# fritzsedlazeck/Sniffles

Measured on AMD Instinct MI355X. Metric: SV-signatures clustered/sec (clustering + calling + QC + genotype + INS consensus), higher is better.
Workload: dtype int32/f64

## Files before the change

sniffles_amd/csrc/snf_fused.h:

```cpp
#pragma once
#include "snf_stage_final.h"
#include "snf_stage_cluster.h"
#include "snf_stage_call.h"

namespace snf {

template <int K>
SNF_D void block_exscan256(const unsigned long long (&val)[K], unsigned long long (&excl)[K], unsigned long long (&tot)[K],
                           unsigned long long* lds) {
  const int tid = threadIdx.x, lane = tid & 63, wid = tid >> 6;
  unsigned long long incl[K];
#pragma unroll
  for (int k = 0; k < K; k++) {
    unsigned long long x = val[k];
#pragma unroll
    for (int d = 1; d < 64; d <<= 1) { const unsigned long long y = __shfl_up(x, d, 64); if (lane >= d) x += y; }
    incl[k] = x;
    if (lane == 63) lds[wid * K + k] = x;
  }
  __syncthreads();
#pragma unroll
  for (int k = 0; k < K; k++) {
    unsigned long long base = 0, all = 0;
#pragma unroll
// ... 165 lines not shown
  if (p < n) {
    v.headscan[p] = (uint32_t)off[0];
    if (p == n - 1) { const int64_t nb = (int64_t)(off[0] + val[0]); v.headscan[n] = (uint32_t)nb; v.cnt->n_bins = nb; v.bin_lo[nb] = (int32_t)v.cnt->n_valid; }
    a3_emit(p, v);
  }
}
SNF_FUSED_HEAD(a4k_binstats)
  if (p < n) a4_binstats_body(p, v);
  unsigned long long val[1] = {p < n ? (unsigned long long)v.eligflag[p] : 0ull};
  tile_publish<1>(v, TS_SEEDS, val, lds);
}
SNF_FUSED_HEAD(a7k_seeds)
  unsigned long long val[1] = {p < n ? (unsigned long long)v.eligflag[p] : 0ull}, off[1];
  tile_scan<1>(v, TS_SEEDS, val, off, lds);
  if (p < n) {
    v.eligscan[p] = (uint32_t)off[0];
    if (p == n - 1) { v.eligscan[n] = (uint32_t)(off[0] + val[0]); v.cnt->n_seeds = (int64_t)(off[0] + val[0]); }
    a7_seeds_body(p, v);
  }
}
SNF_FUSED_HEAD(a5k_leadflags)
  if (p < n) a5_leadflags_body(p, v);
  unsigned long long val[2] = {p < n ? (unsigned long long)v.fN[p] : 0ull, p < n ? (unsigned long long)v.fL[p] : 0ull};
  tile_publish<2>(v, TS_LEADS, val, lds);
}
SNF_FUSED_HEAD(a6k_scatter)
  unsigned long long val[2] = {p < n ? (unsigned long long)v.fN[p] : 0ull, p < n ? (unsigned long long)v.fL[p] : 0ull}, off[2];
  tile_scan<2>(v, TS_LEADS, val, off, lds);
  if (p < n) {
    v.pN[p] = (uint32_t)off[0]; v.pL[p] = (uint32_t)off[1];
    if (p == n - 1) {
      v.pN[n] = (uint32_t)(off[0] + val[0]); v.pL[n] = (uint32_t)(off[1] + val[1]);
      v.cnt->NF = (int64_t)(off[0] + val[0]); v.cnt->NLL = (int64_t)(off[1] + val[1]);
    }
    a6_emit(p, v);
  }
}
SNF_FUSED_HEAD(b1k_seedmetrics)
  if (p < n) b1_seedmetrics_body(p, v);
  unsigned long long val[1] = {p < n ? (unsigned long long)v.runflag[p] : 0ull};
  tile_publish<1>(v, TS_RUNS, val, lds);
}
SNF_FUSED_HEAD(b2k_runs)
  unsigned long long val[1] = {p < n ? (unsigned long long)v.runflag[p] : 0ull}, off[1];
  tile_scan<1>(v, TS_RUNS, val, off, lds);
  if (p < n) {
    v.runscan[p] = (uint32_t)off[0];
    if (p == n - 1) { const int64_t nr = (int64_t)(off[0] + val[0]); v.runscan[n] = (uint32_t)nr; v.cnt->n_runs = nr; v.run_first[nr] = (int32_t)v.cnt->n_seeds; }
    b2_emit(p, v);
  }
}
SNF_FUSED_HEAD(c4a_count)
  unsigned long long val[1] = {p < n ? (unsigned long long)v.clflag[p] : 0ull};
  tile_publish<1>(v, TS_CLUSTERS, val, lds);
}
SNF_FUSED_HEAD(c4k_clusters)
  unsigned long long val[1] = {p < n ? (unsigned long long)v.clflag[p] : 0ull}, off[1];
  tile_scan<1>(v, TS_CLUSTERS, val, off, lds);
  if (p < n) {
    v.clscan[p] = (uint32_t)off[0];
    if (p == n - 1) { v.clscan[n] = (uint32_t)(off[0] + val[0]); v.cnt->n_clusters = (int64_t)(off[0] + val[0]); }
    c4_emit(p, v);
  }
}
SNF_FUSED_HEAD(d1bk_rctable)
  unsigned long long val[1] = {p < n ? (unsigned long long)v.rcflag[p] : 0ull}, off[1];
  tile_scan_direct<1>(v, TS_REFINED, val, off, lds);
  if (p < n) {
    v.rcscan[p] = (uint32_t)off[0];
    if (p == n - 1) { v.rcscan[n] = (uint32_t)(off[0] + val[0]); v.cnt->n_rc = (int64_t)(off[0] + val[0]); }
    d1b_emit(p, v);
  }
}
SNF_FUSED_HEAD(d3ck_compact)
  unsigned long long val[1] = {(p < n && p < v.cnt->n_rc) ? (unsigned long long)v.cdflag[p] : 0ull}, off[1];
  tile_scan_direct<1>(v, TS_CALLS, val, off, lds);
  if (p < n) {
    v.cdscan[p] = (uint32_t)off[0];
    if (p == n - 1) { v.cdscan[n] = (uint32_t)(off[0] + val[0]); v.cnt->n_calls = (int64_t)(off[0] + val[0]); }
    d3_compact_emit(p, v);
  }
}

SNF_FUSED_HEAD(d3sk_svid)
  if (p < n) d3_svid_body(p, v);
  unsigned long long val[1] = {p < n ? (unsigned long long)v.rnf[p] : 0ull};
  tile_publish<1>(v, TS_RNAMES, val, lds);
}
SNF_FUSED_HEAD(d3rk_rnames)
  unsigned long long val[1] = {p < n ? (unsigned long long)v.rnf[p] : 0ull}, off[1];
  tile_scan<1>(v, TS_RNAMES, val, off, lds);
  if (p < n) {
    v.rnp[p] = (uint32_t)off[0];
    if (p == n - 1) { const int64_t tot = (int64_t)(off[0] + val[0]); v.rnp[n] = (uint32_t)tot; v.cnt->rn_total = tot; *v.res_rn_total = tot; }
    if (!v.rn_defer) d3_rnames_emit(p, v);
  }
}

SNF_CHAIN_HEAD(b12c_seedruns, TS_RUNS)
  if (p < n) b1_seedmetrics_body(p, v);
  unsigned long long val[1] = {p < n ? (unsigned long long)v.runflag[p] : 0ull}, off[1], tot[1];
  chain_scan<1>(v, TS_RUNS, tile, val, off, tot, lds);
  if (p < n) {
    v.runscan[p] = (uint32_t)off[0];
    if (p == n - 1) { const int64_t nr = (int64_t)tot[0]; v.runscan[n] = (uint32_t)nr; v.cnt->n_runs = nr; v.run_first[nr] = (int32_t)v.cnt->n_seeds; }
    b2_emit(p, v);
  }
}
SNF_CHAIN_HEAD(c4c_clusters, TS_CLUSTERS)
  unsigned long long val[1] = {p < n ? (unsigned long long)v.clflag[p] : 0ull}, off[1], tot[1];
  chain_scan<1>(v, TS_CLUSTERS, tile, val, off, tot, lds);
  if (p < n) {
    v.clscan[p] = (uint32_t)off[0];
    if (p == n - 1) { v.clscan[n] = (uint32_t)tot[0]; v.cnt->n_clusters = (int64_t)tot[0]; }
    c4_emit(p, v);
  }
}
SNF_CHAIN_HEAD(d1bc_rctable, TS_REFINED)
  unsigned long long val[1] = {p < n ? (unsigned long long)v.rcflag[p] : 0ull}, off[1], tot[1];
  chain_scan<1>(v, TS_REFINED, tile, val, off, tot, lds);
  if (p < n) {
    v.rcscan[p] = (uint32_t)off[0];
    if (p == n - 1) { v.rcscan[n] = (uint32_t)tot[0]; v.cnt->n_rc = (int64_t)tot[0]; }
    d1b_emit(p, v);
  }
}
SNF_CHAIN_HEAD(d3cc_compact, TS_CALLS)
  unsigned long long val[1] = {(p < n && p < v.cnt->n_rc) ? (unsigned long long)v.cdflag[p] : 0ull}, off[1], tot[1];
  chain_scan<1>(v, TS_CALLS, tile, val, off, tot, lds);
  if (p < n) {
    v.cdscan[p] = (uint32_t)off[0];
    if (p == n - 1) { v.cdscan[n] = (uint32_t)tot[0]; v.cnt->n_calls = (int64_t)tot[0]; }
    d3_compact_emit(p, v);
  }
}
SNF_CHAIN_HEAD(d3src_svid_rnames, TS_RNAMES)
  if (p < n) d3_svid_body(p, v);
  unsigned long long val[1] = {p < n ? (unsigned long long)v.rnf[p] : 0ull}, off[1], tot[1];
  chain_scan<1>(v, TS_RNAMES, tile, val, off, tot, lds);
  if (p < n) {
    v.rnp[p] = (uint32_t)off[0];
    if (p == n - 1) { v.rnp[n] = (uint32_t)tot[0]; v.cnt->rn_total = (int64_t)tot[0]; *v.res_rn_total = (int64_t)tot[0]; }
    if (!v.rn_defer) d3_rnames_emit(p, v);
  }
}

#define SNF_ALT_K 5
SNF_D void alt_values(const View& v, int64_t i, int64_t nc, unsigned long long (&val)[SNF_ALT_K]) {
  if (i < nc) { val[0] = v.fN[i]; val[1] = v.fL[i]; val[2] = (unsigned long long)v.sz_tab[i]; val[3] = (unsigned long long)v.sz_aln[i]; val[4] = (unsigned long long)v.sz_rd[i]; }
  else { for (int k = 0; k < SNF_ALT_K; k++) val[k] = 0; }
}
__global__ void __launch_bounds__(256) e2a_sizes(const View v, int64_t n_unused) {
  __shared__ unsigned long long lds[4 * SNF_ALT_K];
  const int64_t nc = v.cnt->n_calls;
  const int64_t i = (int64_t)blockIdx.x * 256 + threadIdx.x;
  for (int64_t k = i; k < 4 * 64 * 16; k += (int64_t)gridDim.x * 256) v.stripes[k] = 0;
  e2_best_body(i, v);
  unsigned long long val[SNF_ALT_K], excl[SNF_ALT_K], tot[SNF_ALT_K];
  alt_values(v, i, nc, val);
  block_exscan256<SNF_ALT_K>(val, excl, tot, lds);
  if (threadIdx.x == 0) for (int k = 0; k < SNF_ALT_K; k++) v.tile_sums[(int64_t)k * v.tile_stride + blockIdx.x] = tot[k];
}
__global__ void __launch_bounds__(256) e3b_offsets(const View v, int64_t n_unused) {
  IT_SCOPE(8)
  __shared__ unsigned long long lds[4 * SNF_ALT_K];
  const int64_t nc = v.cnt->n_calls;
  const int64_t i = (int64_t)blockIdx.x * 256 + threadIdx.x;
  if ((int64_t)blockIdx.x * 256 >= nc) return;
  unsigned long long part[SNF_ALT_K], dummy[SNF_ALT_K], prefix[SNF_ALT_K];
#pragma unroll
  for (int k = 0; k < SNF_ALT_K; k++) {
    unsigned long long a = 0;
    for (int64_t j = threadIdx.x; j < (int64_t)blockIdx.x; j += 256) a += v.tile_sums[(int64_t)k * v.tile_stride + j];
    part[k] = a;
  }
  block_exscan256<SNF_ALT_K>(part, dummy, prefix, lds);
  unsigned long long val[SNF_ALT_K], excl[SNF_ALT_K], tot[SNF_ALT_K];
  alt_values(v, i, nc, val);
  block_exscan256<SNF_ALT_K>(val, excl, tot, lds);
  if (i < nc) {
    const unsigned long long o0 = prefix[0] + excl[0], o1 = prefix[1] + excl[1], o2 = prefix[2] + excl[2], o3 = prefix[3] + excl[3],
                             o4 = prefix[4] + excl[4];
    v.pN[i] = (uint32_t)o0; v.pL[i] = (uint32_t)o1; v.sc_tab[i] = (int64_t)o2; v.sc_aln[i] = (int64_t)o3; v.sc_rd[i] = (int64_t)o4;
    if (i == nc - 1) {
      v.pN[nc] = (uint32_t)(o0 + val[0]); v.pL[nc] = (uint32_t)(o1 + val[1]);
      v.sc_tab[nc] = (int64_t)(o2 + val[2]); v.sc_aln[nc] = (int64_t)(o3 + val[3]); v.sc_rd[nc] = (int64_t)(o4 + val[4]);
      v.cnt->alt_total = (int64_t)(o0 + val[0]); v.cnt->n_cons = (int64_t)(o1 + val[1]);
      v.cnt->tab_total = (int64_t)(o2 + val[2]); v.cnt->aln_total = (int64_t)(o3 + val[3]); v.cnt->n_cons_reads = (int64_t)(o4 + val[4]);
      alt_decide(v, (int64_t)(o0 + val[0]));
    }
    e3_emit(i, v);
  }
}

}
```

sniffles_amd/csrc/snf_knobs.h:

```cpp
#pragma once
#include <climits>
#include <cstdlib>
#include <cstring>
#include <string>

namespace snf {

constexpr int KNOB_UNSET = INT_MIN;
inline bool env_set(const char* name) { return getenv(name) != nullptr; }
inline int env_int(const char* name, int unset) { const char* e = getenv(name); return e ? atoi(e) : unset; }
inline int env_pos(const char* name, int other) { const int v = env_int(name, 0); return v > 0 ? v : other; }
inline bool env_on(const char* name) { return env_int(name, 0) != 0; }
inline bool env_is(const char* name, const char* value) { const char* e = getenv(name); return e && strcmp(e, value) == 0; }
inline std::string env_str(const char* name) { const char* e = getenv(name); return e ? e : ""; }

struct BatchKnobs {
  bool wave_path = !env_set("SNF_NO_WAVE");
  bool fuse = !env_set("SNF_NO_FUSE");
  bool sort64 = env_set("SNF_SORT64");
  bool prefilter = !env_set("SNF_NO_PREFILTER");
  bool pf_spread = env_int("SNF_PF_SPREAD", 0) == 1;
  bool winfront = !env_set("SNF_NO_WINFRONT");
  int win_bits = env_int("SNF_WIN_BITS", 0);
  int win_bits_max = [] { const int v = env_int("SNF_WIN_BITS_MAX", 10); return v >= 6 && v <= 12 ? v : 10; }();
  bool w4_split = env_on("SNF_W4_SPLIT");
  bool pool_slices = !env_set("SNF_NO_POOL_SLICES");
  int fuse_copy = env_set("SNF_FUSE_COPY") ? env_on("SNF_FUSE_COPY") : -1;
  bool merge_reread = env_on("SNF_MERGE_REREAD");
  int run_gap = env_int("SNF_RUN_GAP", KNOB_UNSET);
  int chain = env_set("SNF_CHAIN") ? env_on("SNF_CHAIN") : env_set("SNF_NO_CHAIN") ? 0 : -1;
  int graph = env_set("SNF_GRAPH") ? env_on("SNF_GRAPH") : env_set("SNF_NO_GRAPH") ? 0 : -1;
  int heavy_n = env_int("SNF_HEAVY_N", 24);
  int e1_batch = env_int("SNF_E1_BATCH", 64);
  bool big_stage = !env_set("SNF_NO_BIG_STAGE");
  bool cov_exact = env_set("SNF_COV_EXACT");
  bool d4_thread = env_is("SNF_D4", "thread");
  bool d1_groups = !env_set("SNF_NO_D1_GROUPS");
  bool d2_groups = !env_set("SNF_NO_D2_GROUPS");
  bool d2_mid = env_set("SNF_D2_MID");
  bool rn_defer = !env_set("SNF_NO_RN_DEFER");
  bool rn_fuse = !env_set("SNF_NO_RN_FUSE");
  int grid_mult = env_int("SNF_GRID_MULT", 2);
  int grid_div = env_pos("SNF_GRID_DIV", 1);
  int occ_d2 = env_int("SNF_OCC_D2", 5);
  int occ_e1 = env_int("SNF_OCC_E1", 5);
  int occ_s = env_int("SNF_OCC_S", 5);
  int cons_nw = env_int("SNF_CONS_NW", 1);
  int cons_large_nw = env_int("SNF_CONS_LARGE_NW", 4);
  int cons_grid_mult = env_int("SNF_CONS_GRID_MULT", KNOB_UNSET);
  int cons_small_grid = env_pos("SNF_CONS_SMALL_GRID", 65536);
  int cons_order = env_int("SNF_CONS_ORDER", -1);
  bool serial = env_set("SNF_SERIAL");
  int f4_grid = env_pos("SNF_F4_GRID", 2048);
  bool large_prio = env_on("SNF_LARGE_PRIO");
  int readprep = env_int("SNF_READPREP", 1);
  bool readprep_each_pass = env_set("SNF_READPREP_EACH_PASS");
  int stage_out = env_int("SNF_STAGE_OUT", -1);
  bool stage_copy_kernel = env_is("SNF_STAGE_COPY", "kernel");
  bool alt_hbm = env_set("SNF_ALT_HBM");
  bool prof = env_set("SNF_PROF");
  bool timing = !env_set("SNF_NO_TIMING");
  bool timeline = env_set("SNF_TIMELINE");
  bool time_all = env_set("SNF_TIME_ALL");
  int time_every = env_int("SNF_TIME_EVERY", 8);
  std::string wg_trace_file = env_str("SNF_WG_TRACE_FILE");
};

struct ProcessKnobs {
  int pace = env_int("SNF_PACE", 1);
  double pace_frac = getenv("SNF_PACE_FRAC") ? atof(getenv("SNF_PACE_FRAC")) : 0.25;
  bool chain_gate = env_on("SNF_CHAIN_GATE");
  int gpu_slots = env_int("SNF_GPU_SLOTS", 0);
  size_t stage_arena_floor = getenv("SNF_STAGE_ARENA_MB") ? (size_t)atoll(getenv("SNF_STAGE_ARENA_MB")) << 20 : 0;
  bool slab_cache = !env_set("SNF_NO_SLAB_CACHE");
  bool stream_pool = !env_set("SNF_NO_STREAM_POOL");
  bool roctx = env_on("SNF_ROCTX");
  int upload_threads = env_set("SNF_UPLOAD_THREADS") ? env_pos("SNF_UPLOAD_THREADS", 1) : 0;
};
inline const ProcessKnobs& process_knobs() { static const ProcessKnobs k; return k; }

struct ExtractKnobs {
  bool thread_form = env_set("SNF_EXTRACT_THREAD");
  int waves = env_int("SNF_EXTRACT_WAVES", 4);
  int grid_cap = env_set("SNF_EXTRACT_GRID") ? env_pos("SNF_EXTRACT_GRID", 1) : (1 << 22);
  bool xtrace_emit = env_is("SNF_XTRACE_PASS", "emit");
  std::string xtrace_out = env_str("SNF_XTRACE_OUT");
};

struct BgzfKnobs {
  bool thread_form = env_set("SNF_BGZF_THREAD");
  int grid_cap = env_set("SNF_BGZF_GRID") ? env_pos("SNF_BGZF_GRID", 1) : (1 << 20);
};

struct BaiKnobs {
  bool thread_form = env_set("SNF_BAI_THREAD");
  int grid_cap = env_set("SNF_BAI_GRID") ? env_pos("SNF_BAI_GRID", 1) : (1 << 20);
};

struct DeflateKnobs {
  int grid_cap = env_set("SNF_DEFLATE_GRID") ? env_pos("SNF_DEFLATE_GRID", 1) : (1 << 20);
  int max_bits = [] { const int v = env_int("SNF_DEFLATE_MAXBITS", 15); return v >= 9 && v <= 15 ? v : 15; }();
};

struct FastaKnobs {
  int grid_cap = env_set("SNF_FASTA_GRID") ? env_pos("SNF_FASTA_GRID", 1) : (1 << 20);
};

struct CombineKnobs {
  bool thread_form = env_set("SNF_COMBINE_THREAD");
};

}
```

sniffles_amd/csrc/snf_lib.hip:

```cpp
#include "snf_stage_final.h"
#include "snf_wave_refine.h"
#include "snf_wave_cons.h"
#include "snf_fused.h"
#include "snf_stage_window.h"
#include "snf_stage_out.h"
#include "snf_wave_call.h"
#include "snf_wave_call_g.h"
#include "snf_wave_refine_g.h"
#include "snf_ctx.h"

#include <rocprim/device/device_radix_sort.hpp>
#include <rocprim/device/device_scan.hpp>

#include <fcntl.h>
#include <sys/file.h>
#include <unistd.h>

#include <atomic>
#include <map>
#include <tuple>
#include <cmath>
#include <ctime>
#include <memory>
#include <mutex>
// ... 1320 lines not shown
    prim_exscan<uint32_t>(b, v.runflag, v.runscan, N + 1, "scan_runs");
    LAUNCH_Q(b2_runs, v, N, N * 4);
    LAUNCH(c1_mergeruns, v, N, N * 8);
    LAUNCH_Q(c2_validate, v, N, 0);
    LAUNCH_Q(c3_serial, v, 8 * (int64_t)T, 0);
    prim_exscan<uint32_t>(b, v.clflag, v.clscan, N + 1, "scan_clusters");
    LAUNCH_Q(c4_clusters, v, N, N * 4);
    dzero(b, v.rcflag, sizeof(uint32_t) * (N + 1));
    }
    if (b->k.readprep == 3) fork_mark(b);
    if (v.wave_path && b->k.d1_groups) {
      { ClassFork _f(b);
        Scope _s(b, "d1g_refine8", N * 36 / 3);
        hipLaunchKernelGGL((v.fuse_defer ? d1g_refine<8, true> : d1g_refine<8, false>), dim3(b->slots_d1w), dim3(64), 0, b->cur, v, (int64_t)0);
        SNF_HIP(hipGetLastError()); }
      { Scope _s(b, "d1w_refine", N * 36 - N * 36 / 3);
        v.d1_from_list = 1;
        hipLaunchKernelGGL((v.fuse_defer ? d1w_refine<true> : d1w_refine<false>), dim3(b->slots_d1w), dim3(64), 0, b->cur, v, (int64_t)0);
        v.d1_from_list = 0;
        SNF_HIP(hipGetLastError()); }
      join_classes(b);
    } else if (v.wave_path) {
      Scope _s(b, "d1w_refine", N * 36);
      hipLaunchKernelGGL((v.fuse_defer ? d1w_refine<true> : d1w_refine<false>), dim3(b->slots_d1w), dim3(64), 0, b->cur, v, (int64_t)0);
      SNF_HIP(hipGetLastError());
    }
    if (!(v.wave_path && b->fused)) LAUNCH_Q(d1_refine, v, N, v.wave_path ? 0 : N * 36);
    b->skipped_big[0] = b->skipped_big[1] = b->skipped_big[2] = false;
    if (v.wave_path && b->have_big_hist && b->hist_big[0] == 0) b->skipped_big[0] = true;
    else if (v.wave_path) {
      Scope _s(b, "x_big_refine", 0);
      hipLaunchKernelGGL(x_big<0>, dim3(b->slots_big), dim3(64), 0, b->cur, v, (int64_t)0);
      SNF_HIP(hipGetLastError());
    }
  }
  if (b->k.readprep == 1 || b->k.readprep == 3) enqueue_read_prep(b);
  if (N > 0) {
    if (b->fused && v.chain_on) CHAIN(d1bc_rctable, N);
    else if (b->fused) FUSED(d1bk_rctable, N);
    else {
      prim_exscan<uint32_t>(b, v.rcflag, v.rcscan, N + 1, "scan_refined");
      LAUNCH_Q(d1b_rctable, v, N, N * 4);
    }
    const bool call_forks = v.wave_path && b->k.d2_groups && classes_beside(b);
    if (v.fuse_defer && !call_forks) enqueue_fuse_copy(b, nullptr);
    if (v.wave_path && b->k.d2_groups) {
      const bool ph = b->cfg.phase != 0;
      { ClassFork _f(b);
        Scope _s(b, "d2g_call8", N * 32 / 3);
        if (ph) hipLaunchKernelGGL((d2g_call<8, 4, true>), dim3(b->slots_d2w), dim3(64), 0, b->cur, v, (int64_t)0);
        else hipLaunchKernelGGL((d2g_call<8, 4, false>), dim3(b->slots_d2w), dim3(64), 0, b->cur, v, (int64_t)0);
        SNF_HIP(hipGetLastError()); }
      if (v.fuse_defer && call_forks) enqueue_fuse_copy(b, b->ev_cls_fork);
      const bool mid = b->k.d2_mid;
      if (mid) { Scope _s(b, "d2g_call32", 0);
        if (ph) hipLaunchKernelGGL((d2g_call<32, 4, true>), dim3(b->slots_d2w), dim3(64), 0, b->cur, v, (int64_t)0);
        else hipLaunchKernelGGL((d2g_call<32, 4, false>), dim3(b->slots_d2w), dim3(64), 0, b->cur, v, (int64_t)0);
        SNF_HIP(hipGetLastError()); }
      { Scope _s(b, "d2w_call", N * 32 - N * 32 / 3);
        v.d2_from_list = mid ? 2 : 1;
        hipLaunchKernelGGL(b->k_d2w, dim3(b->slots_d2w), dim3(64), 0, b->cur, v, (int64_t)0);
        v.d2_from_list = 0;
        SNF_HIP(hipGetLastError()); }
      join_classes(b);
    } else if (v.wave_path) {
      Scope _s(b, "d2w_call", N * 32);
      hipLaunchKernelGGL(b->k_d2w, dim3(b->slots_d2w), dim3(64), 0, b->cur, v, (int64_t)0);
      SNF_HIP(hipGetLastError());
    }
    if (!(v.wave_path && b->fused)) LAUNCH_Q(d2_call, v, N, v.wave_path ? 0 : N * 32);
    if (v.wave_path && b->have_big_hist && b->hist_big[1] == 0) b->skipped_big[1] = true;
    else if (v.wave_path) {
      Scope _s(b, "x_big_call", 0);
      hipLaunchKernelGGL(x_big<1>, dim3(b->slots_big), dim3(64), 0, b->cur, v, (int64_t)0);
      SNF_HIP(hipGetLastError());
    }
    if (b->fused && v.chain_on) CHAIN(d3cc_compact, N);
    else if (b->fused) FUSED(d3ck_compact, N);
    else {
      prim_exscan<uint32_t>(b, v.cdflag, v.cdscan, N + 1, "scan_calls");
      LAUNCH_Q(d3_compact, v, N, 0);
    }
  }
  LAUNCH_Q(d3_taskoff, v, tail_threads(v), 0);
  SNF_HIP(hipEventRecord(b->ev_counts, b->stream));
  if (b->k.readprep == 2) enqueue_read_prep(b);
  fork_mark(b);
  if (b->fused) {
    {
      SNF_HIP(hipStreamWaitEvent(b->stream4, b->ev_fork, 0));
      hipStream_t prev = b->cur; b->cur = b->stream4;
      if (N > 0 && v.chain_on) { Scope _s(b, "d3_rnames", 0); CHAIN(d3src_svid_rnames, N); }
      else if (N > 0) {
        FUSED(d3sk_svid, N);
        { Scope _s(b, "d3_rnames", 0); FUSED(d3rk_rnames, N); }
      } else *b->h_rn_total = 0;
      SNF_HIP(hipEventRecord(b->ev_rn, b->stream4));
      b->cur = prev;
    }
    SideStream side(b);
    if (N > 0) launch_coverage(b, N);
  } else
  {
    SideStream side(b);
    if (N > 0) {
      LAUNCH_Q(d3_svid, v, N, 0);
      prim_exscan<uint32_t>(b, v.rnf, v.rnp, N + 1, "scan_rnames");
      LAUNCH(d3_rnames, v, N, 0);
    } else *b->h_rn_total = 0;
    SNF_HIP(hipEventRecord(b->ev_rn, b->cur));
    if (N > 0) launch_coverage(b, N);
  }
  b->res_current = false;
  v.out_valid = 0;
  b->side_open = true;
}

void join_fourth(snf_batch_impl* b) {
  SNF_HIP(hipEventRecord(b->ev_join4, b->stream4));
  SNF_HIP(hipStreamWaitEvent(b->stream, b->ev_join4, 0));
  b->side_open = false;
}
void join_open_candidates(snf_batch_impl* b) {
  if (!b->side_open || b->capturing) return;
  join_side(b);
  join_fourth(b);
}
void full_sync(snf_batch_impl* b) {
  join_side(b);
  join_fourth(b);
  if (!b->res_current) { LAUNCH_Q(z1_results, b->v, tail_threads(b->v), 0); b->res_current = true; }
  dsync(b);
}

void ensure_cap(snf_batch_impl* b, int64_t need, int64_t& cap, void** p, size_t elem) {
  if (need <= cap && *p) return;
  if (*p) dfree_one(b, *p);
  cap = need + need / 4 + 64;
  *p = dalloc_own<uint8_t>(b, (size_t)cap * elem);
}

void enqueue_rnames_late(snf_batch_impl* b, bool all) {
  View& v = b->v;
  if (b->rn_state == 0 || (b->rn_state == 2 && !all) || v.NS <= 0) return;
  const int keep = v.rn_defer;
  v.rn_defer = all ? 2 : 1;
  { Scope _s(b, "d3_rnames_late", 0);
    unsigned grid = (unsigned)((v.NS / 4 + 255) / 256) + 1u; if (grid > 4096u) grid = 4096u;
    hipLaunchKernelGGL(d3lk_rnames_late, dim3(grid), dim3(256), 0, b->cur, v, (int64_t)0);
    SNF_HIP(hipGetLastError()); }
  v.rn_defer = keep;
  b->rn_state = all ? 0 : 2;
}

void enqueue_output_head(snf_batch_impl* b) {
  SNF_TRACE("F: output stage (filter, rank, records + read names)");
  View& v = b->v;
  const int64_t NS = v.NS;
  const bool rn_all = !((v.out_mode & SNF_OUT_EXECUTE) && !v.cfg.no_qc);
  const bool rn_src = b->rn_state == 1 && !rn_all && b->fused && NS > 0 && NS <= ((int64_t)1 << 22) * 256 && b->k.rn_fuse;
  if (!rn_src) enqueue_rnames_late(b, rn_all);
  if (b->fused && NS <= ((int64_t)1 << 22) * 256) {
    const unsigned grid = (unsigned)((NS + 255) / 256) > 0u ? (unsigned)((NS + 255) / 256) : 1u;
    FUSED(f1k_outflags, NS > 0 ? NS : 1);
    FUSED(f2k_outscan, NS > 0 ? NS : 1);
    if ((v.out_mode & SNF_OUT_EXECUTE) && v.cfg.sort) {
      Scope _s(b, "f3_rank", 0);
// ... 518 lines not shown
    }
    noff[T] = w; b->r_off = noff; nc = w;
  }
  for (int64_t i = 0; i < nc; i++) { calls[i].alt_len = -1; calls[i].alt_off = 0; }
  collect_timings(b);
  out->n_calls = nc; out->calls = calls;
  out->alt_pool_len = 0; out->alt_pool = (const uint8_t*)calls;
  out->rnames_len = rn_total; out->rnames = rn;
  out->n_tasks = T; out->task_status = b->r_status.data(); out->task_call_off = b->r_off.data();
  out->coverage_average_total = b->r_cov.data();
  b->pass_idle = true;
}

void do_add_task(snf_batch_impl* b, const snf_task_input_t* t) {
  if (b->uploaded) fail("snf_batch_add_task after snf_batch_upload");
  int64_t n = t->n_leads, r = t->n_reads;
  if (n < 0 || r < 0 || t->contig_len < 0 || t->seq_pool_len < 0) fail("negative sizes in task input");
  if (n > 0 && (!t->ref_start || !t->ref_end || !t->qry_start || !t->qry_end || !t->svlen || !t->read_len || !t->qname_id ||
                !t->read_id || !t->ps_rank || !t->mate_contig || !t->mate_ref_start || !t->seq_len || !t->seq_off || !t->nm ||
                !t->svtype || !t->strand || !t->mapq || !t->source || !t->hap || !t->is_sa || !t->bnd_is_first || !t->bnd_is_reverse))
    fail("null lead column");
  if (r > 0 && (!t->read_start || !t->read_end || !t->read_hp)) fail("null read column");
  if (t->seq_pool_len > 0 && !t->seq_pool) fail("null sequence pool");
  int64_t ntr = t->n_tr > 0 ? t->n_tr : 0;
  int32_t pm = INT32_MIN;
  for (int64_t i = 0; i < ntr; i++) {
    b->h_trs.push_back(t->tr_start[i]); b->h_tre.push_back(t->tr_end[i]);
    if (t->tr_end[i] > pm) pm = t->tr_end[i];
    b->h_trp.push_back(pm);
  }
  b->h_has_tr.push_back(ntr > 0 ? 1 : 0);
  {
    const int64_t nn = t->n_nmask > 0 ? t->n_nmask : 0;
    if (nn > 0 && (!t->nmask_start || !t->nmask_end)) fail("null mask arrays");
    int32_t prev = 0;
    for (int64_t i = 0; i < nn; i++) {
      const int32_t a = t->nmask_start[i], e = t->nmask_end[i];
      if (a < prev || e <= a || e > t->contig_len) fail("mask intervals must be sorted, disjoint, non-empty and inside the contig (leadprov.py:434-441)");
      b->h_nms.push_back(a); b->h_nme.push_back(e); prev = e;
    }
    b->h_nm_off.push_back((int64_t)b->h_nms.size());
  }
  b->h_lead_off.push_back(b->h_lead_off.back() + n);
  b->h_read_off.push_back(b->h_read_off.back() + r);
  b->h_pool_off.push_back(b->h_pool_off.back() + t->seq_pool_len);
  b->h_tr_off.push_back((int64_t)b->h_trs.size());
  b->tasks.push_back(*t);
  b->task_on_device.push_back(0);
}

}

namespace {
void do_consensus_batch(int device, int klen, const uint8_t* seq_pool, int64_t seq_pool_len, int64_t n_problems,
                        const int64_t* best_off, const int32_t* best_len, const int32_t* skip, const int32_t* skip_rep, const int64_t* others_index,
                        const int64_t* others_off, const int32_t* others_len, uint8_t* out_pool, const int64_t* out_off) {
    if (n_problems <= 0) return;
    if (!seq_pool || !best_off || !best_len || !skip || !others_index || !others_off || !others_len || !out_pool || !out_off)
      fail("snf_consensus_batch: null argument");
    int nd = 0;
    if (hipGetDeviceCount(&nd) != hipSuccess || nd <= 0 || device < 0 || device >= nd) fail("no such HIP device");
    SNF_HIP(hipSetDevice(device));
    if (klen < 1 || klen > 8) fail("snf_consensus_batch: klen must be 1..8 (a k-mer is compared as one 64-bit word)");
    const bool has_dash = seq_pool_len > 0 && memchr(seq_pool, '-', (size_t)seq_pool_len) != nullptr;
    const int64_t np = n_problems, n_reads = others_index[np];
    std::vector<ConsDesc> descs((size_t)np);
    std::vector<int32_t> lists[8];
    std::vector<int64_t> generic;
    Counts hc{};
    int64_t aln_total = 0, alt_total = 0;
    for (int64_t p = 0; p < np; p++) {
      const int64_t L = best_len[p]; const int64_t no = others_index[p + 1] - others_index[p];
      if (L < 0 || no < 0 || best_off[p] < 0 || best_off[p] + L > seq_pool_len) fail("best sequence outside the pool");
      if (out_off[p + 1] - out_off[p] != L) fail("out_off must be the prefix sums of best_len");
      if (skip[p] < 1 || (skip_rep && skip_rep[p] < 1)) fail("sampling steps must be >= 1 (range() of the reference raises on 0)");
      for (int64_t k = others_index[p]; k < others_index[p + 1]; k++)
        if (others_len[k] < 0 || others_off[k] < 0 || others_off[k] + others_len[k] > seq_pool_len) fail("other sequence outside the pool");
      const int cls = (has_dash || (skip_rep && skip_rep[p] != skip[p])) ? 0 : cons_class_of(1, klen, skip[p], L, (int32_t)no);
      if (cls == 0) { generic.push_back(p); continue; }
      ConsDesc d{};
      d.best_off = best_off[p]; d.alt_off = out_off[p]; d.aln_off = aln_total; d.read_off = others_index[p];
      d.L = (int32_t)L; d.n_others = (int32_t)no; d.skip = skip[p]; d.cls = cls;
      descs[(size_t)p] = d;
      int lid = cls;
      if (cls == 2) { const int64_t work = no * L; lid = work >= 32768 ? 2 : work >= 16384 ? 3 : work >= 8192 ? 4 : 5; }
      else if (cls == 4) lid = 7;
      lists[lid].push_back((int32_t)p); hc.n_cls[lid]++;
      aln_total += no * L;
    }
    alt_total = out_off[np];
    std::vector<void*> frees;
    auto dev = [&](size_t bytes) { void* q = nullptr; SNF_HIP(hipMalloc(&q, bytes ? bytes : 1)); frees.push_back(q); return q; };
    auto up = [&](const void* h, size_t bytes) { void* q = dev(bytes); if (bytes) SNF_HIP(hipMemcpy(q, h, bytes, hipMemcpyHostToDevice)); return q; };
    struct Guard { std::vector<void*>& f; ~Guard() { for (void* q : f) (void)hipFree(q); } } guard{frees};
    View v{};
    v.cfg.consensus_kmer_len = klen;
    v.wave_path = 1;
    uint8_t* dpool = (uint8_t*)dev((size_t)seq_pool_len + 32);
    SNF_HIP(hipMemset(dpool, 0, (size_t)seq_pool_len + 32));
    if (seq_pool_len) SNF_HIP(hipMemcpy(dpool, seq_pool, (size_t)seq_pool_len, hipMemcpyHostToDevice));
    v.pool = dpool; v.pool_len = seq_pool_len; v.pool_cap = seq_pool_len + 32;
    v.alt_pool = (uint8_t*)dev((size_t)alt_total + 16);
    if ((int64_t)generic.size() < np) {
    v.cdesc = (ConsDesc*)up(descs.data(), descs.size() * sizeof(ConsDesc));
    for (int k = 1; k < 6; k++) v.cls_list[k] = (int32_t*)up(lists[k].data(), lists[k].size() * sizeof(int32_t));
    lists[7].resize((size_t)np, 0);
    v.cls_list[7] = (int32_t*)up(lists[7].data(), lists[7].size() * sizeof(int32_t));
    v.cnt = (Counts*)up(&hc, sizeof(Counts));
    v.crl_off = (int64_t*)up(others_off, (size_t)n_reads * sizeof(int64_t));
    v.crl_len = (int32_t*)up(others_len, (size_t)n_reads * sizeof(int32_t));
    v.aln = (uint8_t*)dev((size_t)aln_total + 16);
    v.aln_kept_w = (uint8_t*)dev((size_t)n_reads + 16);
    v.stripes = (unsigned long long*)dev(4 * 64 * 16 * sizeof(unsigned long long));
    SNF_HIP(hipMemset(v.stripes, 0, 4 * 64 * 16 * sizeof(unsigned long long)));
    const int64_t n_small = (int64_t)hc.n_cls[1], n_large = (int64_t)(hc.n_cls[2] + hc.n_cls[3] + hc.n_cls[4] + hc.n_cls[5]);
    if (n_large > 0) hipLaunchKernelGGL((K_CONS_LARGE), dim3((unsigned)(n_large < 16384 ? n_large : 16384)), dim3(256), 0, 0, v, (int64_t)0);
    if (n_small > 0) hipLaunchKernelGGL((K_CONS_SMALL(5)), dim3((unsigned)(n_small < 16384 ? n_small : 16384)), dim3(256), 0, 0, v, (int64_t)0);
    hipLaunchKernelGGL((K_CONS_ROWS), dim3((unsigned)(np < 4096 ? np : 4096)), dim3(256), 0, 0, v, (int64_t)0);
    SNF_HIP(hipGetLastError());
    }
    if (!generic.empty()) {
      const int64_t ng = (int64_t)generic.size();
      std::vector<CallX> cx((size_t)ng);
      std::vector<int32_t> ccall((size_t)ng), fi, flen, sk((size_t)ng), skr((size_t)ng);
      std::vector<int64_t> foff, roff((size_t)ng + 1), toff((size_t)ng + 1), tsz((size_t)ng), aoff((size_t)ng + 1);
      std::vector<uint32_t> pn((size_t)np + 1);
      std::vector<CallX> call_all((size_t)np);
      for (int64_t p = 0; p < np; p++) { pn[(size_t)p] = (uint32_t)out_off[p]; CallX x{}; x.do_cons = 0; x.best = -1; x.cons_id = -1; call_all[(size_t)p] = x; }
      pn[(size_t)np] = (uint32_t)out_off[np];
      if (out_off[np] >= ((int64_t)1 << 32)) fail("snf_consensus_batch: more than 4 GB of output");
      int64_t r_tot = 0, t_tot = 0, a_tot = 0;
      for (int64_t k = 0; k < ng; k++) {
        const int64_t p = generic[(size_t)k], L = best_len[p], no = others_index[p + 1] - others_index[p];
        CallX x{};
        x.flo = (int32_t)fi.size(); x.fn = (int32_t)(no + 1); x.best = x.flo; x.n_others = (int32_t)no; x.do_cons = 1; x.cons_id = (int32_t)k;
        fi.push_back((int32_t)fi.size()); flen.push_back((int32_t)L); foff.push_back(best_off[p]);
        for (int64_t q = others_index[p]; q < others_index[p + 1]; q++) { fi.push_back((int32_t)fi.size()); flen.push_back(others_len[q]); foff.push_back(others_off[q]); }
        if (fi.size() >= ((size_t)1 << 31)) fail("snf_consensus_batch: too many sequences");
        call_all[(size_t)p] = x; ccall[(size_t)k] = (int32_t)p;
        sk[(size_t)k] = skip[p]; skr[(size_t)k] = skip_rep ? skip_rep[p] : skip[p];
        const int64_t npos = cons_npos(L, klen, skr[(size_t)k]);
        int64_t hs = 16; while (hs < 2 * npos + 2) hs <<= 1;
        roff[(size_t)k] = r_tot; toff[(size_t)k] = t_tot; tsz[(size_t)k] = hs; aoff[(size_t)k] = a_tot;
        r_tot += no; t_tot += hs; a_tot += no * L;
      }
      roff[(size_t)ng] = r_tot; toff[(size_t)ng] = t_tot; aoff[(size_t)ng] = a_tot;
      View g{};
      g.cfg.consensus_kmer_len = klen; g.wave_path = 1; g.cons_thread_only = 1;
      g.pool = dpool; g.pool_len = seq_pool_len; g.pool_cap = seq_pool_len + 32;
      Counts gc{}; gc.n_cons = ng; gc.n_cons_reads = r_tot; gc.alt_total = out_off[np]; gc.n_calls = np; gc.alt_in_pinned = 0;
      g.cnt = (Counts*)up(&gc, sizeof(Counts));
      g.cons_call = (int32_t*)up(ccall.data(), ccall.size() * 4);
      g.callx = (CallX*)up(call_all.data(), call_all.size() * sizeof(CallX));
      g.F_seq_len = (int32_t*)up(flen.data(), flen.size() * 4); g.F_seq_off = (int64_t*)up(foff.data(), foff.size() * 8);
      g.FI = (int32_t*)up(fi.data(), fi.size() * 4);
      g.cons_read_off = (int64_t*)up(roff.data(), roff.size() * 8); g.cons_tab_off = (int64_t*)up(toff.data(), toff.size() * 8);
      g.cons_tab_sz = (int64_t*)up(tsz.data(), tsz.size() * 8); g.cons_aln_off = (int64_t*)up(aoff.data(), aoff.size() * 8);
      g.cons_skip_arr = (int32_t*)up(sk.data(), sk.size() * 4); g.cons_skiprep_arr = (int32_t*)up(skr.data(), skr.size() * 4);
      g.pN = (uint32_t*)up(pn.data(), pn.size() * 4);
      g.tab_key = (uint64_t*)dev((size_t)t_tot * 8); g.tab_pos = (int32_t*)dev((size_t)t_tot * 4); g.tab_state = (uint8_t*)dev((size_t)t_tot);
      g.aln = (uint8_t*)dev((size_t)a_tot + 16); g.aln_kept = (uint8_t*)dev((size_t)r_tot + 16);
      g.cr_call = (int32_t*)dev((size_t)r_tot * 4 + 4); g.cr_read = (int32_t*)dev((size_t)r_tot * 4 + 4);
      g.alt_pool = v.alt_pool;
      auto grid = [](int64_t n) { return dim3((unsigned)((n + 255) / 256)); };
      hipLaunchKernelGGL(e4_anchor, grid(ng), dim3(256), 0, 0, g, ng);
      if (r_tot > 0) hipLaunchKernelGGL(e5_align, grid(r_tot), dim3(256), 0, 0, g, r_tot);
      if (out_off[np] > 0) hipLaunchKernelGGL(e6_vote, grid(out_off[np]), dim3(256), 0, 0, g, out_off[np]);
      SNF_HIP(hipGetLastError());
    }
// ... 585 lines not shown
```

sniffles_amd/csrc/snf_stage_final.h:

```cpp
#pragma once
#include "snf_stage_call.h"

namespace snf {

#define SNF_PS_NULL_CODE 0x7fffffff

struct LeadIter {
  const View& v; const CallX& x; int32_t k;
  SNF_HD LeadIter(const View& v_, const CallX& x_) : v(v_), x(x_), k(-1) {}
  SNF_HD bool next(int32_t* slot, uint32_t* orig) {
    for (k++; k < x.fn; k++) {
      int32_t s = v.FI[x.flo + k];
      if (v.F_sel[s]) { *slot = s; *orig = (uint32_t)v.F_orig[s]; return true; }
    }
    return false;
  }
};

struct LeadAgg {
  int nstrands;
  int64_t close_edge;
  int hp_val; int64_t hp_support, hp_other;
  int32_t ps_val; int64_t ps_support, ps_other;
  const double* nm_row;
// ... 380 lines not shown
    int64_t cnt = 0;
    const NmGet get{v, x, g.nm_row};
    for (int64_t i = 0; i < n; i++) { double nm = get.raw(i); if (nm == nm) cnt++; }
    sv_nm = np_pairwise_sum<DEPTH>(get, n) / (double)cnt;
  }
  if (sv_nm > cfg.genotype_error || n <= 3) return;
  if (!c.ph_set || !c.ph_hp_pass) return;
  int hp = c.ph_hp;
  if (hp != 1 && hp != 2) return;
  int32_t h = v.cl_head[x.cluster];
  int32_t b = v.seed_bin[h];
  int32_t sv_reads = v.bin_hap[3 * b + hp];
  int32_t all_reads = hapref_count(v, task, hp, (int64_t)v.seed_start[h] / v.cfg.cluster_binsize);
  if (all_reads == 0) return;
  if ((double)sv_reads / (double)all_reads >= 0.75) {
    if (c.filter == SNF_F_MOSAIC_VAF) { c.filter = SNF_F_PASS; c.gt_b = 1; c.qc = 1; }
  }
}

SNF_HD void store_final_fields(snf_call_t& dst, const snf_call_t& c) {
  dst.qc = c.qc; dst.filter = c.filter;
  dst.gt_set = c.gt_set; dst.gt_a = c.gt_a; dst.gt_b = c.gt_b; dst.gt_gq = c.gt_gq; dst.gt_dr = c.gt_dr; dst.gt_dv = c.gt_dv;
  dst.gt_hp = c.gt_hp; dst.gt_ps = c.gt_ps; dst.vaf = c.vaf;
  dst.ph_set = c.ph_set; dst.ph_hp = c.ph_hp; dst.ph_ps = c.ph_ps; dst.ph_hp_support = c.ph_hp_support;
  dst.ph_ps_support = c.ph_ps_support; dst.ph_hp_pass = c.ph_hp_pass; dst.ph_ps_pass = c.ph_ps_pass;
}

template <int DEPTH>
SNF_HD void finalize_call(const View& v, snf_call_t& c, const CallX& x, const LeadAgg& g, int task) {
  const snf_config_t& cfg = v.cfg;
  c.qc = c.qc && qc_sv(v, c, g);
  if (!cfg.mosaic && c.qc) c.qc = c.qc && qc_sv_support(c, v.t_cov_avg[task], cfg);
  int hp_ret = -1, ps_ret = -1;
  if (cfg.phase) phase_sv(v, c, g, &hp_ret, &ps_ret);
  genotype_sv(v, c, hp_ret, ps_ret);
  c.qc = c.qc && qc_sv_post_annotate(v, c, g, task);
  bool phasing_rescue = c.svtype != SNF_BND && iabs64(c.svlen) <= cfg.dev_maxsvlen_extra &&
                        c.support >= (int)((double)cfg.dev_minreads_extra * 0.60);
  if (cfg.phase && !c.qc && phasing_rescue) rescue_phasing<DEPTH>(v, c, x, task, g);
}

SNF_HD void e1_finalize_body(int64_t i, const View& v) {
  if (i >= v.cnt->n_calls) return;
  snf_call_t& cref = v.calls[i];
  int task = cref.task_index;
  if (v.t_status[task] != SNF_TASK_OK) return;
  const CallX x = v.callx[i];
  if (v.wave_path && (x.fn <= 64 || v.big_wave)) return;
  snf_call_t c = cref;
  LeadAgg g;
  collect_agg(v, x, task, &g);
  finalize_call<26>(v, c, x, g, task);
  store_final_fields(cref, c);
}

SNF_HD int64_t cons_npos(int64_t L, int klen, int skip) { int64_t m = L - klen; return m <= 0 ? 0 : (m + skip - 1) / skip; }
SNF_HD int cons_skip(const snf_config_t& cfg, int64_t L) {
  return cfg.consensus_kmer_skip_base + (int)((double)L * cfg.consensus_kmer_skip_seqlen_mult);
}

#define SNF_CONS_SMALL_L 384
#define SNF_CONS_LARGE_L 8192
SNF_HD int cons_class_of(int wave_path, int klen, int skip, int64_t L, int32_t n_others) {
  if (!wave_path || klen > 7 || klen < 1 || skip < 1 || L >= 65000) return 0;
  int64_t npos = cons_npos(L, klen, skip);
  if (npos <= 120 && n_others <= 64 && L <= SNF_CONS_SMALL_L && skip <= 7) return 1;
  if (npos <= 500 && n_others <= 254 && L <= SNF_CONS_LARGE_L) return 2;
  if (npos <= 500 && n_others <= 512) return 4;
  return 0;
}
SNF_HD int cons_class(const View& v, int64_t L, int32_t n_others) {
  if (v.cons_thread_only) return 0;
  return cons_class_of(v.wave_path, v.cfg.consensus_kmer_len, cons_skip(v.cfg, L), L, n_others);
}
SNF_HD int cons_skip_reads(const View& v, int64_t cid, int64_t L) { return v.cons_skip_arr ? v.cons_skip_arr[cid] : cons_skip(v.cfg, L); }
SNF_HD int cons_skip_anchors(const View& v, int64_t cid, int64_t L) { return v.cons_skiprep_arr ? v.cons_skiprep_arr[cid] : cons_skip(v.cfg, L); }
SNF_HD bool cons_wave_eligible(const View& v, int64_t L, int32_t n_others) { return cons_class(v, L, n_others) != 0; }

SNF_HD uint8_t* alt_base(const View& v) { return v.cnt->alt_in_pinned ? v.alt_pin : v.alt_pool; }
SNF_HD void alt_decide(const View& v, int64_t alt_total) {
  v.cnt->alt_in_pinned = (!(v.out_mode & SNF_OUT_DEVICE) && v.alt_pin && alt_total <= v.alt_pin_cap) ? 1 : 0;
}

SNF_HD void e2_best_body(int64_t i, const View& v) {
  const int64_t nc = v.cnt->n_calls;
  if (i == 0) {
    v.fN[nc] = 0; v.fL[nc] = 0; v.sz_tab[nc] = 0; v.sz_aln[nc] = 0; v.sz_rd[nc] = 0;
    for (int k = 0; k < 8; k++) v.cnt->n_cls[k] = 0;
    v.cnt->n_cons_fallback = 0;
    if (nc == 0) alt_decide(v, 0);
  }
  if (i >= nc) return;
  v.fN[i] = 0; v.fL[i] = 0; v.sz_tab[i] = 0; v.sz_aln[i] = 0; v.sz_rd[i] = 0;
  snf_call_t& c = v.calls[i];
  CallX& x = v.callx[i];
  x.cons_id = -1;
  if (c.svtype != SNF_INS || v.cfg.symbolic || v.t_status[c.task_index] != SNF_TASK_OK || x.best < 0) { x.best = -1; x.n_others = 0; x.do_cons = 0; return; }
  const int32_t best = x.best;
  const int64_t L = v.F_seq_len[best];
  c.alt_len = (int32_t)L;
  v.fN[i] = (uint32_t)L;
  v.fL[i] = 1u;
  if (x.do_cons) {
    v.sz_aln[i] = (int64_t)x.n_others * L;
    v.sz_rd[i] = x.n_others;
    if (!cons_wave_eligible(v, L, x.n_others)) {
      int64_t npos = cons_npos(L, v.cfg.consensus_kmer_len, cons_skip(v.cfg, L));
      int64_t hs = 16; while (hs < 2 * npos + 2) hs <<= 1;
      v.sz_tab[i] = hs;
    }
  }
}

SNF_HD int64_t class_list_slot(const View& v, int lid) {
#if defined(__HIP_DEVICE_COMPILE__)
  int64_t slot = 0;
  for (int c = 0; c < 8; c++) {
    const unsigned long long m = __ballot(lid == c);
    if (lid == c) {
      const int lane = (int)__lane_id();
      const int leader = __builtin_ctzll(m);
      unsigned long long base = 0;
      if (lane == leader) base = atomic_add_u64(&v.cnt->n_cls[c], (unsigned long long)__builtin_popcountll(m));
      base = __shfl(base, leader, 64);
      slot = (int64_t)base + __builtin_popcountll(m & ((1ull << lane) - 1ull));
    }
  }
  return slot;
#else
  return (int64_t)atomic_add_u64(&v.cnt->n_cls[lid], 1ull);
#endif
}

SNF_HD void e3_emit(int64_t i, const View& v);
SNF_HD void e3_conslist_body(int64_t i, const View& v) {
  const int64_t nc = v.cnt->n_calls;
  if (i == 0) {
    v.cnt->alt_total = v.pN[nc]; v.cnt->n_cons = v.pL[nc];
    v.cnt->tab_total = v.sc_tab[nc]; v.cnt->aln_total = v.sc_aln[nc]; v.cnt->n_cons_reads = v.sc_rd[nc];
    alt_decide(v, (int64_t)v.pN[nc]);
  }
  if (i >= nc) return;
  e3_emit(i, v);
}
SNF_HD void e3_emit(int64_t i, const View& v) {
  snf_call_t& c = v.calls[i];
  CallX& x = v.callx[i];
  if (c.alt_len < 0) return;
  c.alt_off = v.pN[i]; x.alt_off = v.pN[i];
  uint32_t cid = v.pL[i];
  x.cons_id = (int32_t)cid;
  v.cons_call[cid] = (int32_t)i;
  v.cons_tab_off[cid] = v.sc_tab[i]; v.cons_tab_sz[cid] = v.sz_tab[i];
  v.cons_aln_off[cid] = v.sc_aln[i]; v.cons_read_off[cid] = v.sc_rd[i];
  if (v.sz_tab[i] > 0) atomic_add_u64((unsigned long long*)&v.cnt->n_cons_fallback, 1ull);
  if (!v.wave_path) return;
  ConsDesc d;
  d.L = v.F_seq_len[x.best]; d.best_off = v.F_seq_off[x.best]; d.alt_off = x.alt_off; d.aln_off = v.sc_aln[i];
  d.read_off = x.flo;
  d.n_others = x.n_others; d.skip = cons_skip(v.cfg, d.L);
  d.cls = x.do_cons ? (cons_class(v, d.L, x.n_others) ? cons_class(v, d.L, x.n_others) : 3) : 0;
  v.cdesc[cid] = d;
  int lid = d.cls;
  if (d.cls == 2) {
    const int64_t work = (int64_t)d.n_others * d.L;
    lid = work >= 32768 ? 2 : work >= 16384 ? 3 : work >= 8192 ? 4 : 5;
  } else if (d.cls == 3) lid = 6;
  else if (d.cls == 4) lid = 7;
  const int64_t slot = class_list_slot(v, lid);
  if (lid != 6) v.cls_list[lid][slot] = (int32_t)cid;
}

SNF_HD uint64_t kmer_key(const uint8_t* s, int klen) {
  uint64_t k = 0;
  for (int i = 0; i < klen; i++) k = (k << 8) | s[i];
  return k;
}
SNF_HD int64_t kmer_slot(uint64_t key, int64_t hs) { return (int64_t)((key * 0x9E3779B97F4A7C15ull) >> 40) & (hs - 1); }

SNF_HD void e4_anchor_body(int64_t cid, const View& v) {
  if (cid >= v.cnt->n_cons) return;
  int32_t ci = v.cons_call[cid];
  const CallX& x = v.callx[ci];
  int64_t L = v.F_seq_len[x.best];
  if (!x.do_cons) return;
  int64_t r0 = v.cons_read_off[cid];
  for (int32_t r = 0; r < x.n_others; r++) { v.cr_call[r0 + r] = (int32_t)cid; v.cr_read[r0 + r] = r; }
  if (cons_wave_eligible(v, L, x.n_others)) return;
  const uint8_t* B = v.pool + v.F_seq_off[x.best];
  int klen = v.cfg.consensus_kmer_len, skip = cons_skip_anchors(v, cid, L);
  int64_t t0 = v.cons_tab_off[cid], hs = v.cons_tab_sz[cid];
  uint64_t* key = v.tab_key + t0; int32_t* pos = v.tab_pos + t0; uint8_t* st = v.tab_state + t0;
  for (int64_t p = 0; p < hs; p++) st[p] = 0;
  for (int64_t i = 0; i < L - klen; i += skip) {
    uint64_t kk = kmer_key(B + i, klen);
    int64_t p = kmer_slot(kk, hs);
    while (st[p] && key[p] != kk) p = (p + 1) & (hs - 1);
    if (st[p] == 0) { st[p] = 1; key[p] = kk; pos[p] = (int32_t)i; }
    else st[p] = 2;
  }
}

SNF_HD void e5_align_body(int64_t j, const View& v) {
  if (j >= v.cnt->n_cons_reads) return;
  int32_t cid = v.cr_call[j], ridx = v.cr_read[j];
  int32_t ci = v.cons_call[cid];
  const CallX& x = v.callx[ci];
  if (cons_wave_eligible(v, v.F_seq_len[x.best], x.n_others)) return;
  int32_t slot = -1, seen = 0;
  for (int32_t k = 0; k < x.fn; k++) {
    int32_t s = v.FI[x.flo + k];
    if (v.F_seq_len[s] < 0 || s == x.best) continue;
    if (seen == ridx) { slot = s; break; }
    seen++;
  }
  int64_t L = v.F_seq_len[x.best];
  const uint8_t* B = v.pool + v.F_seq_off[x.best];
  const uint8_t* S = v.pool + v.F_seq_off[slot];
  int64_t SL = v.F_seq_len[slot];
  int klen = v.cfg.consensus_kmer_len, skip = cons_skip_reads(v, cid, L), maxshift = klen;
  int64_t t0 = v.cons_tab_off[cid], hs = v.cons_tab_sz[cid];
  const uint64_t* key = v.tab_key + t0; const int32_t* pos = v.tab_pos + t0; const uint8_t* st = v.tab_state + t0;
  uint8_t* row = v.aln + v.cons_aln_off[cid] + (int64_t)ridx * L;
  bool have_last = false; int64_t last_i = 0, last_j = 0, clen = 0, span = 0;
  for (int64_t jj = 0; jj < SL - klen; jj += skip) {
    uint64_t kk = kmer_key(S + jj, klen);
    int64_t p = kmer_slot(kk, hs);
    while (st[p] && key[p] != kk) p = (p + 1) & (hs - 1);
    if (st[p] != 1) continue;
    int64_t i = pos[p];
    if (iabs64(i - jj) > maxshift) continue;
    if (have_last && i <= last_i) continue;
    if (!have_last) {
      if (jj > 0) { for (int64_t q = 0; q < i; q++) row[q] = '-'; clen = i; }
    } else {
      int64_t fwd_i = i - last_i, fwd_j = jj - last_j;
      if (clen + fwd_j > L) fwd_j = L - clen;
      if (fwd_i == fwd_j && fwd_j > 0) {
        span += jj - last_j;
        int64_t m = 0;
        for (int64_t l = 1; l <= jj - last_j; l++) if (S[last_j + l] == B[last_i + l]) m++;
        double ident = (double)m / (double)(jj - last_j);
        if (ident >= 0.5) for (int64_t q = 0; q < fwd_j; q++) row[clen + q] = S[last_j + q];
        else for (int64_t q = 0; q < fwd_j; q++) row[clen + q] = '-';
        clen += fwd_j;
      } else if (fwd_j > 0) { for (int64_t q = 0; q < fwd_j; q++) row[clen + q] = '-'; clen += fwd_j; }
    }
    have_last = true; last_i = i; last_j = jj;
  }
  for (int64_t q = clen; q < L; q++) row[q] = '-';
  for (int64_t hh = 0; hh < L;) {
// ... 95 lines not shown
```

Baseline: 3.480 billion.

## Compute per-task call offsets with wave-parallel binary search and pass scan offsets directly

Replaces the thread-per-element d3_taskoff with a one-wavefront-per-task kernel. It locates task boundaries and the first BND call through a 64-way ballot-based lower-bound search, and copies the Counts block to the result buffer in the same kernel. The e3 emit path now receives its offsets in registers from the scan instead of re-reading the pN/pL/sc_* arrays it just wrote, and e2a blocks beyond n_calls skip the block scan. Class-list selection is moved into shared helpers used by both device and host code. The search cost is roughly T×log64(nc) global reads, and a thread fallback is kept behind an env knob.

```diff
diff --git a/sniffles_amd/csrc/snf_fused.h b/sniffles_amd/csrc/snf_fused.h
--- a/sniffles_amd/csrc/snf_fused.h
+++ b/sniffles_amd/csrc/snf_fused.h
@@ -271,6 +271,43 @@
   }
 }
 
+template <class Below>
+SNF_D int64_t wave_lower_bound(int64_t lo, int64_t hi, Below below) {
+  const int lane = (int)(threadIdx.x & 63);
+  while (lo < hi) {
+    const int64_t step = (hi - lo + 63) / 64;
+    const int64_t p = lo + (int64_t)(lane + 1) * step - 1;
+    const int k = __builtin_popcountll(__ballot(p < hi && below(p)));
+    const int64_t pk = lo + (int64_t)(k + 1) * step - 1;
+    lo += (int64_t)k * step;
+    hi = pk < hi ? pk : hi;
+  }
+  return lo;
+}
+__global__ void __launch_bounds__(64) d3w_taskoff(const View v, int64_t n_unused) {
+  const int64_t t = blockIdx.x, nc = v.cnt->n_calls;
+  if (t <= v.T) {
+    const int64_t lo = wave_lower_bound(0, nc, [&](int64_t p) { return (int64_t)v.calls[p].task_index < t; });
+    if (threadIdx.x == 0) v.t_call_off[t] = lo;
+    if (t < v.T) {
+      const int64_t hi = wave_lower_bound(lo, nc, [&](int64_t p) { return (int64_t)v.calls[p].task_index < t + 1; });
+      const int64_t a = wave_lower_bound(lo, hi, [&](int64_t p) { return v.calls[p].svtype < SNF_BND; });
+      if (threadIdx.x == 0) {
+        v.t_status[t] = SNF_TASK_OK; v.t_stale_end[t] = 0;
+        if (a < hi && v.calls[a].svtype == SNF_BND) {
+          if (a == lo) v.t_status[t] = SNF_TASK_ERR_UNBOUND_END;
+          else {
+            const snf_call_t& p = v.calls[a - 1];
+            v.t_stale_end[t] = p.svtype == SNF_INS ? p.pos + 1 : (int32_t)((int64_t)p.pos + iabs64(p.svlen));
+          }
+        }
+      }
+    }
+  }
+  const unsigned long long* s = (const unsigned long long*)v.cnt; unsigned long long* d = (unsigned long long*)v.res_cnt;
+  for (size_t k = (size_t)blockIdx.x * 64 + threadIdx.x; k < sizeof(Counts) / 8; k += (size_t)gridDim.x * 64) d[k] = s[k];
+}
+
 SNF_FUSED_HEAD(d3sk_svid)
   if (p < n) d3_svid_body(p, v);
   unsigned long long val[1] = {p < n ? (unsigned long long)v.rnf[p] : 0ull};
@@ -345,6 +382,7 @@
   const int64_t i = (int64_t)blockIdx.x * 256 + threadIdx.x;
   for (int64_t k = i; k < 4 * 64 * 16; k += (int64_t)gridDim.x * 256) v.stripes[k] = 0;
   e2_best_body(i, v);
+  if ((int64_t)blockIdx.x * 256 >= nc) return;
   unsigned long long val[SNF_ALT_K], excl[SNF_ALT_K], tot[SNF_ALT_K];
   alt_values(v, i, nc, val);
   block_exscan256<SNF_ALT_K>(val, excl, tot, lds);
@@ -378,8 +416,9 @@
       v.cnt->tab_total = (int64_t)(o2 + val[2]); v.cnt->aln_total = (int64_t)(o3 + val[3]); v.cnt->n_cons_reads = (int64_t)(o4 + val[4]);
       alt_decide(v, (int64_t)(o0 + val[0]));
     }
-    e3_emit(i, v);
-  }
-}
-
-}
+    const AltOffsets o = {(uint32_t)o0, (uint32_t)o1, (int64_t)o2, (int64_t)val[2], (int64_t)o3, (int64_t)o4};
+    e3_emit(i, v, o);
+  }
+}
+
+}
diff --git a/sniffles_amd/csrc/snf_knobs.h b/sniffles_amd/csrc/snf_knobs.h
--- a/sniffles_amd/csrc/snf_knobs.h
+++ b/sniffles_amd/csrc/snf_knobs.h
@@ -35,6 +35,7 @@
   bool big_stage = !env_set("SNF_NO_BIG_STAGE");
   bool cov_exact = env_set("SNF_COV_EXACT");
   bool d4_thread = env_is("SNF_D4", "thread");
+  bool taskoff_thread = env_is("SNF_TASKOFF", "thread");
   bool d1_groups = !env_set("SNF_NO_D1_GROUPS");
   bool d2_groups = !env_set("SNF_NO_D2_GROUPS");
   bool d2_mid = env_set("SNF_D2_MID");
diff --git a/sniffles_amd/csrc/snf_lib.hip b/sniffles_amd/csrc/snf_lib.hip
--- a/sniffles_amd/csrc/snf_lib.hip
+++ b/sniffles_amd/csrc/snf_lib.hip
@@ -1426,7 +1426,12 @@
       LAUNCH_Q(d3_compact, v, N, 0);
     }
   }
-  LAUNCH_Q(d3_taskoff, v, tail_threads(v), 0);
+  if (v.wave_path && b->fused && !b->k.taskoff_thread) {
+    const unsigned grid = (unsigned)(v.T + 1 > 2 ? v.T + 1 : 2);
+    if (b->time_all) { Scope _s(b, "d3_taskoff", 0); hipLaunchKernelGGL(d3w_taskoff, dim3(grid), dim3(64), 0, b->cur, v, (int64_t)0); }
+    else hipLaunchKernelGGL(d3w_taskoff, dim3(grid), dim3(64), 0, b->cur, v, (int64_t)0);
+    SNF_HIP(hipGetLastError());
+  } else LAUNCH_Q(d3_taskoff, v, tail_threads(v), 0);
   SNF_HIP(hipEventRecord(b->ev_counts, b->stream));
   if (b->k.readprep == 2) enqueue_read_prep(b);
   fork_mark(b);
@@ -2111,9 +2116,7 @@
       d.best_off = best_off[p]; d.alt_off = out_off[p]; d.aln_off = aln_total; d.read_off = others_index[p];
       d.L = (int32_t)L; d.n_others = (int32_t)no; d.skip = skip[p]; d.cls = cls;
       descs[(size_t)p] = d;
-      int lid = cls;
-      if (cls == 2) { const int64_t work = no * L; lid = work >= 32768 ? 2 : work >= 16384 ? 3 : work >= 8192 ? 4 : 5; }
-      else if (cls == 4) lid = 7;
+      const int lid = alt_list_of_class(cls, L, (int32_t)no);
       lists[lid].push_back((int32_t)p); hc.n_cls[lid]++;
       aln_total += no * L;
     }
diff --git a/sniffles_amd/csrc/snf_stage_final.h b/sniffles_amd/csrc/snf_stage_final.h
--- a/sniffles_amd/csrc/snf_stage_final.h
+++ b/sniffles_amd/csrc/snf_stage_final.h
@@ -486,6 +486,20 @@
   v.cnt->alt_in_pinned = (!(v.out_mode & SNF_OUT_DEVICE) && v.alt_pin && alt_total <= v.alt_pin_cap) ? 1 : 0;
 }
 
+SNF_HD int alt_class(const View& v, int do_cons, int64_t L, int32_t n_others) {
+  if (!do_cons) return 0;
+  const int cls = cons_class(v, L, n_others);
+  return cls ? cls : 3;
+}
+SNF_HD int alt_list_of_class(int cls, int64_t L, int32_t n_others) {
+  if (cls == 2) {
+    const int64_t work = (int64_t)n_others * L;
+    return work >= 32768 ? 2 : work >= 16384 ? 3 : work >= 8192 ? 4 : 5;
+  }
+  return cls == 3 ? 6 : cls == 4 ? 7 : cls;
+}
+SNF_HD int alt_list_id(const View& v, int do_cons, int64_t L, int32_t n_others) { return alt_list_of_class(alt_class(v, do_cons, L, n_others), L, n_others); }
+
 SNF_HD void e2_best_body(int64_t i, const View& v) {
   const int64_t nc = v.cnt->n_calls;
   if (i == 0) {
@@ -536,7 +550,8 @@
 #endif
 }
 
-SNF_HD void e3_emit(int64_t i, const View& v);
+struct AltOffsets { uint32_t alt_off, cid; int64_t tab_off, tab_sz, aln_off, rd_off; };
+SNF_HD void e3_emit(int64_t i, const View& v, const AltOffsets& o);
 SNF_HD void e3_conslist_body(int64_t i, const View& v) {
   const int64_t nc = v.cnt->n_calls;
   if (i == 0) {
@@ -545,32 +560,28 @@
     alt_decide(v, (int64_t)v.pN[nc]);
   }
   if (i >= nc) return;
-  e3_emit(i, v);
-}
-SNF_HD void e3_emit(int64_t i, const View& v) {
+  const AltOffsets o = {v.pN[i], v.pL[i], v.sc_tab[i], v.sz_tab[i], v.sc_aln[i], v.sc_rd[i]};
+  e3_emit(i, v, o);
+}
+SNF_HD void e3_emit(int64_t i, const View& v, const AltOffsets& o) {
   snf_call_t& c = v.calls[i];
   CallX& x = v.callx[i];
   if (c.alt_len < 0) return;
-  c.alt_off = v.pN[i]; x.alt_off = v.pN[i];
-  uint32_t cid = v.pL[i];
+  c.alt_off = o.alt_off; x.alt_off = o.alt_off;
+  const uint32_t cid = o.cid;
   x.cons_id = (int32_t)cid;
   v.cons_call[cid] = (int32_t)i;
-  v.cons_tab_off[cid] = v.sc_tab[i]; v.cons_tab_sz[cid] = v.sz_tab[i];
-  v.cons_aln_off[cid] = v.sc_aln[i]; v.cons_read_off[cid] = v.sc_rd[i];
-  if (v.sz_tab[i] > 0) atomic_add_u64((unsigned long long*)&v.cnt->n_cons_fallback, 1ull);
+  v.cons_tab_off[cid] = o.tab_off; v.cons_tab_sz[cid] = o.tab_sz;
+  v.cons_aln_off[cid] = o.aln_off; v.cons_read_off[cid] = o.rd_off;
+  if (o.tab_sz > 0) atomic_add_u64((unsigned long long*)&v.cnt->n_cons_fallback, 1ull);
   if (!v.wave_path) return;
   ConsDesc d;
-  d.L = v.F_seq_len[x.best]; d.best_off = v.F_seq_off[x.best]; d.alt_off = x.alt_off; d.aln_off = v.sc_aln[i];
+  d.L = v.F_seq_len[x.best]; d.best_off = v.F_seq_off[x.best]; d.alt_off = o.alt_off; d.aln_off = o.aln_off;
   d.read_off = x.flo;
   d.n_others = x.n_others; d.skip = cons_skip(v.cfg, d.L);
-  d.cls = x.do_cons ? (cons_class(v, d.L, x.n_others) ? cons_class(v, d.L, x.n_others) : 3) : 0;
+  d.cls = alt_class(v, x.do_cons, d.L, x.n_others);
   v.cdesc[cid] = d;
-  int lid = d.cls;
-  if (d.cls == 2) {
-    const int64_t work = (int64_t)d.n_others * d.L;
-    lid = work >= 32768 ? 2 : work >= 16384 ? 3 : work >= 8192 ? 4 : 5;
-  } else if (d.cls == 3) lid = 6;
-  else if (d.cls == 4) lid = 7;
+  const int lid = alt_list_id(v, x.do_cons, d.L, x.n_others);
   const int64_t slot = class_list_slot(v, lid);
   if (lid != 6) v.cls_list[lid][slot] = (int32_t)cid;
 }
```

Measured after the change: 3.529 billion, median of 6. 1.4% higher.
